# cjcliffe/CubicSDR

Measured on AMD Instinct MI355X. Metric: IQ MS/s sustained @ N demods + FFT size, higher is better.
Workload: dtype f32; 1 GPU; C3: 256 mixed NBFM/AM/USB demods, 61.44 MS/s complex-float IQ, firpfbch M=122, 65536-pt spectrum FFT (internal 131072) over every sample; blocks_per_batch=128, block_len=1024068, n_demods=256, fft_size=65536, audio_samples_per_batch=26215768, streams=1

## Files before the change

cubicsdr_amd/csrc/csdr_bank.hip:

```cpp
#include <algorithm>
#include <cstdlib>
#include <cmath>
#include <map>
#include <memory>

#define CSDR_TU_BANK 1
#include "csdr_objects.hpp"
#include "kernels_fms.hpp"

using namespace csdr;

static int bank_arm_bank(csdr_bank *b, const design::MsresampPlan &p, int *idx) {
    uint32_t key;
    memcpy(&key, &p.rate_arb, 4);
    auto it = b->arm_index.find(key);
    if (it != b->arm_index.end()) { *idx = it->second; return CSDR_OK; }
    const int i = (int)b->arm_index.size();
    b->arms_host.insert(b->arms_host.end(), p.arms.begin(), p.arms.end());
    const size_t need = b->arms_host.size();
    if (need > b->arms.cap) {
        if (int rc = b->ctx->sync_all()) return rc;
        if (int rc = b->arms.reserve(std::max(need, b->arms.cap * 2 + (size_t)kArms * kArmTaps * 8))) return rc;
        CSDR_HIP_TRY(hipMemcpy(b->arms.p, b->arms_host.data(), need * sizeof(float), hipMemcpyHostToDevice));
    } else {
        CSDR_HIP_TRY(hipMemcpy(b->arms.p + (size_t)i * kArms * kArmTaps, p.arms.data(), p.arms.size() * sizeof(float), hipMemcpyHostToDevice));
    }
    b->arm_index[key] = i;
    *idx = i;
    return CSDR_OK;
}

extern "C" int csdr_bank_create(csdr_ctx *ctx, int max_demods, int max_blocks, csdr_bank **out) {
    DeviceScope dev__(ctx);
    if (!ctx || !out || max_demods <= 0 || max_blocks <= 0) return fail(CSDR_EINVAL, "bad argument");
    std::unique_ptr<csdr_bank> b(new csdr_bank());
    b->ctx = ctx; b->max_demods = max_demods; b->max_blocks = max_blocks;
    b->slots.resize(max_demods);
    if (int rc = b->cfgs.reserve(max_demods)) return rc;
    b->off_lists = ((size_t)max_demods * sizeof(SlotDyn) + 15) & ~(size_t)15;
    b->off_plans = (b->off_lists + (6 * (size_t)max_demods + 8 * 32) * sizeof(int) + 15) & ~(size_t)15;
    b->table_bytes = (b->off_plans + (size_t)max_demods * (max_blocks + 1) * sizeof(BlockPlan) + 255) & ~(size_t)255;
// ... 437 lines not shown
    }
    CSDR_HIP_TRY(hipEventRecord(b->stage_ev[ring], fetch_on_post ? c->lanes[LANE_POST] : st));
    b->stage_used[ring] = true;
    if (fetch_on_post) CSDR_HIP_TRY(hipStreamWaitEvent(st, b->stage_ev[ring], 0));
    else if (post->ctx != c || !c->same(LANE_POST, LANE_FE)) {
        if (post->ctx != c) CSDR_HIP_TRY(hipEventRecord(post->ev_ready[pk], post->ctx->lanes[LANE_POST]));
        CSDR_HIP_TRY(hipStreamWaitEvent(st, post->ev_ready[pk], 0));
    }
    const int64_t total = (int64_t)NB * Bc;
    const int fe_slots = std::max(1, c->wg_slots(demod_frontend_s<5, 2048, true>, kFeThreads + 64, fes_lds_bytes<5, 2048>()));
    auto ranges_for = [&](int n_slots) {
        int P = (int)std::max<int64_t>(1, std::min<int64_t>(total / std::max<int64_t>(4096, 4 * (int64_t)warm_max), 4096));
        const int per_slot = fe_slots / std::max(1, n_slots) - 1;
        if (per_slot >= 1) {
            P = std::max(P, (int)std::min<int64_t>(total / std::max<int64_t>(2048, (int64_t)warm_max), 4096));
            P = std::min(P, per_slot);
        }
        else {
            const int rounds = (n_slots * 2 + fe_slots - 1) / fe_slots;
            P = std::max(1, std::min(P, rounds * fe_slots / std::max(1, n_slots) - 1));
        }
        return P;
    };
    size_t fe_lds = 0;
    for (int i = 0; i < grp_n[0]; ++i) fe_lds = std::max(fe_lds, fe_lds_bytes((int)b->slots[grp_h[grp_off[0] + i]].iq.S));
    const int cap_stream = (max_n_iq_ag + kSsbWarm + 64 + 3) & ~3;
    const int cap_cw = max_cw_audio ? ((max_cw_audio + 4 * kHilbM + 64 + 3) & ~3) : 0;
    bool any_dsb = false;
    for (int i = 0; i < n_ag; ++i) any_dsb = any_dsb || b->slots[ag_list_h[i]].prm.modem == CSDR_MODEM_DSB;
    const size_t dsb_lds = any_dsb ? 1024 * sizeof(float) + (size_t)(max_n_iq_ag + 64) * sizeof(float2) : 0;
    const size_t cw_lds = cap_cw ? ((size_t)kCwIqWin + 2 * (size_t)cap_cw) * sizeof(float2) : 0;
    const size_t modem_lds = std::max(std::max((size_t)4 * cap_stream * sizeof(float), cw_lds), dsb_lds) + 64;
    int hist_need = 2 * kArmTaps;
    for (int i = 0; i < n_run; ++i) {
        const SlotHost &s = b->slots[slot_list_h[i]];
        if (is_fe_only(s.prm.modem) || s.prm.modem == CSDR_MODEM_IQ) continue;
        const int aS = (int)s.au.S;
        int64_t lo = 0, need;
        if (s.au.interp) {
            for (int st = aS - 1; st >= 0; --st) lo = (lo >> 1) - (2 * (int)s.au.m[st] - 1);
            need = ((-lo * (int64_t)s.au.step) >> 24) + kArmTaps + 8;
        } else {
            lo = -(int64_t)(kArmTaps - 1);
            for (int e = aS - 1; e >= 0; --e) lo = 2 * lo - (4 * (int)s.au.m[aS - 1 - e] - 2);
            need = -lo + (1 << aS) + 8;
        }
        hist_need = std::max<int>(hist_need, (int)need);
    }
    const int cap_win = (max_n_iq + std::min(hist_need, kDHist) + 64 + 3) & ~3;
    const int cap_out = (std::max(max_n_audio + 32 * max_aS + 64, cap_win / 2 + 64) + 3) & ~3;
    const size_t audio_lds = (size_t)(2 * cap_out + cap_win) * sizeof(float) + 64;
    constexpr size_t kLdsPerWorkgroup = 160 * 1024;
    if (modem_lds > kLdsPerWorkgroup || audio_lds > kLdsPerWorkgroup)
        return reject(fail(CSDR_EUNSUPPORTED, "%d IQ / %d audio samples per block need %zu / %zu bytes of LDS (limit %zu)", max_n_iq, max_n_audio, modem_lds, audio_lds, kLdsPerWorkgroup));
    const int fms_blk = (max_n_iq_fms + 4 * kHilbM + 4 + 3) & ~3, fms_au = (max_n_au_fms + 4 + 3) & ~3;
    const size_t fms_pre_lds = (size_t)fms_blk * sizeof(float), fms_pll_lds = 1024 * sizeof(float) + (size_t)fms_blk * (sizeof(float2) + sizeof(uint32_t)),
                 fms_mix_lds = (size_t)2 * (fms_blk + 4 * kHilbM) * sizeof(float),
                 fms_out_lds = ((size_t)2 * (fms_au + kFmsFirMax) + kFmsFirMax) * sizeof(float) + 64;
    if (n_fms && std::max(std::max(fms_pre_lds, fms_pll_lds), std::max(fms_mix_lds, fms_out_lds)) > kLdsPerWorkgroup)
        return reject(fail(CSDR_EUNSUPPORTED, "FM stereo: %d IQ samples per block need more LDS than a workgroup has", max_n_iq_fms));
    const bool fused1 = NB == 1 && n_fms == 0;
    const size_t want[8] = {fe_lds, modem_lds, audio_lds, n_fms ? fms_pre_lds : 0, n_fms ? fms_pll_lds : 0, n_fms ? fms_mix_lds : 0, n_fms ? fms_out_lds : 0,
                            fused1 ? std::max(modem_lds, audio_lds) : 0};
    const void *fn[8] = {(const void *)demod_frontend, (const void *)demod_modem, (const void *)demod_audio_interp,
                         (const void *)fms_pre, (const void *)fms_pll, (const void *)fms_mix, (const void *)fms_out, (const void *)demod_modem_audio1};
    for (int k = 0; k < 8; ++k)
        if (want[k] > 64 * 1024 && want[k] > b->lds_attr[k]) {
            CSDR_HIP_TRY(hipFuncSetAttribute(fn[k], hipFuncAttributeMaxDynamicSharedMemorySize, (int)want[k]));
            b->lds_attr[k] = want[k];
        }
    const dim3 grid(std::max(1, n_audio_run), NB);
    const int audio_threads = kAudioThreads;
    const float2 *chan_out = post_buf(post, pk);
    const int *grp_d = lists_d + 2 * (size_t)b->max_demods;
    if (grp_n[0] > 0)
        CSDR_LAUNCH(c, LANE_FE, KID_FE_GENERIC, demod_frontend, dim3(ranges_for(grp_n[0]), grp_n[0]), dim3(kFeThreads), fe_lds, b->cfgs.p, dyns_d, grp_d + grp_off[0],
                    chan_out, post->chan_stride, total, b->arms.p, c->sintab.p);
#define CSDR_FE_S(S_, CH_)                                                                                                              \
    if (grp_n[S_] > 0)                                                                                                                  \
        CSDR_LAUNCH(c, LANE_FE, KID_FE_S##S_, (demod_frontend_s<S_, CH_>), dim3(16, grp_rows[S_] * (ranges_for(grp_n[S_]) + 1)), dim3(kFeThreads), (fes_lds_bytes<S_, CH_>()), \
                    b->cfgs.p, dyns_d, grp_d + grp_off[S_], chan_out, post->chan_stride, total, b->arms.p, c->sintab.p, grp_rows[S_])
    CSDR_FE_S(3, 2048); CSDR_FE_S(4, 2048);
    if (grp_n[6] > 0) {
        if (merged56)
            CSDR_LAUNCH(c, LANE_FE, KID_FE_S56, (demod_frontend_s56<2048>), dim3(16, grp_rows[6] * (ranges_for(grp_n[6]) + 1)), dim3(kFeThreads + 64), (fes_lds_bytes<6, 2048>()),
                        b->cfgs.p, dyns_d, grp_d + grp_off[6], chan_out, post->chan_stride, total, b->arms.p, c->sintab.p, grp_rows[6]);
        else
            CSDR_LAUNCH(c, LANE_FE, KID_FE_S6, (demod_frontend_s<6, 2048, true>), dim3(16, grp_rows[6] * (ranges_for(grp_n[6]) + 1)), dim3(kFeThreads + 64), (fes_lds_bytes<6, 2048>()),
                        b->cfgs.p, dyns_d, grp_d + grp_off[6], chan_out, post->chan_stride, total, b->arms.p, c->sintab.p, grp_rows[6]);
    }
    if (grp_n[7] > 0) {
        int64_t jmax = 0;
        for (int i = 0; i < grp_n[7]; ++i) jmax = std::max<int64_t>(jmax, b->slots[grp_h[grp_off[7] + i]].last_J);
        const int nchunks = (int)((jmax + kFiChunk - 1) / kFiChunk);
        CSDR_LAUNCH(c, LANE_FE, KID_FE_INTERP, demod_frontend_interp, dim3(nchunks + 1, grp_n[7]), dim3(kFeThreads), kFiLds, b->cfgs.p, dyns_d, grp_d + grp_off[7],
                    chan_out, post->chan_stride, total, b->arms.p, c->sintab.p);
    }
    if (grp_n[5] > 0)
        CSDR_LAUNCH(c, LANE_FE, KID_FE_S5, (demod_frontend_s<5, 2048, true>), dim3(16, grp_rows[5] * (ranges_for(grp_n[5]) + 1)), dim3(kFeThreads + 64), (fes_lds_bytes<5, 2048>()),
                    b->cfgs.p, dyns_d, grp_d + grp_off[5], chan_out, post->chan_stride, total, b->arms.p, c->sintab.p, grp_rows[5]);
#undef CSDR_FE_S
    CSDR_HIP_TRY(hipGetLastError());
    {
        csdr_post *pw = const_cast<csdr_post *>(post);
        if (pw->ctx != c || !c->same(LANE_POST, LANE_FE)) {
            if (pw->n_consumed[pk] >= csdr_post::kMaxConsumers) return fail(CSDR_ERANGE, "too many demodulator banks read one channelizer batch");
            CSDR_HIP_TRY(hipEventRecord(pw->ev_consumed[pk][pw->n_consumed[pk]++], st));
        }
    }
    if (int rc = c->signal(b->ev_fe_done[bpar], LANE_FE, LANE_AUDIO)) return rc;
    if (int rc = c->wait(b->ev_fe_done[bpar], LANE_FE, LANE_AUDIO)) return rc;
    if (int rc = b->audio.wait(st_a)) return rc;
    if (fused1) {
        if (n_audio_run > 0)
            CSDR_LAUNCH(c, LANE_AUDIO, KID_AUDIO, demod_modem_audio1, dim3(n_audio_run), dim3(audio_threads), std::max(modem_lds, audio_lds), b->cfgs.p, dyns_d, lists_d, plans_d,
                        cap_stream, b->mconsts.p, c->sintab.p, b->arms.p, cap_cw, cap_out, cap_win);
    } else {
    if (n_ag > 0)
        CSDR_LAUNCH(c, LANE_AUDIO, KID_MODEM, demod_modem, dim3(NB, n_ag), dim3(audio_threads) , modem_lds, b->cfgs.p, dyns_d, lists_d + b->max_demods,
                    plans_d, NB, cap_stream, b->mconsts.p, c->sintab.p, b->arms.p, cap_cw);
    if (n_ag > 0 && NB > 1)
        CSDR_LAUNCH(c, LANE_AUDIO, KID_GAIN_SCAN, demod_gain_scan, dim3(n_ag), dim3(64), (size_t)(2 * NB + 1) * sizeof(float), b->cfgs.p, dyns_d, lists_d + b->max_demods, plans_d, NB);
    const int *fms_d = lists_d + b->max_demods + fms_off;
    if (n_fms > 0) {
        CSDR_LAUNCH(c, LANE_AUDIO, KID_FMS, fms_pre, dim3(n_fms, NB), dim3(64), fms_pre_lds, b->cfgs.p, dyns_d, fms_d, plans_d, NB, b->mconsts.p);
        CSDR_LAUNCH(c, LANE_AUDIO, KID_FMS, fms_pll, dim3(n_fms), dim3(kModemThreads), fms_pll_lds, b->cfgs.p, fms_d, plans_d, NB, fms_blk, c->sintab.p);
        CSDR_LAUNCH(c, LANE_AUDIO, KID_FMS, fms_mix, dim3(n_fms, NB), dim3(64), fms_mix_lds, b->cfgs.p, dyns_d, fms_d, plans_d, NB, fms_blk - 4 * kHilbM, b->mconsts.p, c->sintab.p);
    }
    if (n_audio_run > 0)
        CSDR_LAUNCH(c, LANE_AUDIO, KID_AUDIO, demod_audio_interp, grid, dim3(audio_threads), audio_lds, b->cfgs.p, dyns_d, lists_d, plans_d, NB,
                    cap_out, cap_win, b->arms.p, 0);
    if (n_fms > 0) {
        CSDR_LAUNCH(c, LANE_AUDIO, KID_AUDIO, demod_audio_interp, dim3(n_fms, NB), dim3(audio_threads), audio_lds, b->cfgs.p, dyns_d, fms_d, plans_d, NB,
                    cap_out, cap_win, b->arms.p, 1);
        CSDR_LAUNCH(c, LANE_AUDIO, KID_FMS_OUT, fms_out, dim3(n_fms, NB), dim3(64), fms_out_lds, b->cfgs.p, dyns_d, fms_d, plans_d, NB, fms_au);
    }
    }
    if (int rc = bank_digital_launch(b, plans_d, NB)) return rc;
    CSDR_HIP_TRY(hipGetLastError());
    if (int rc = c->signal(b->ev_audio_done[bpar], LANE_AUDIO, LANE_FE)) return rc;
    b->audio_pending[bpar] = true;
    if (fetch_on_post) if (int rc = b->tables_read[bpar].release(st_a)) return rc;
    (void)st_a;
    b->seq++;
    return CSDR_OK;
}

int bank_iq_acquire(csdr_bank *b, hipStream_t reader) {
    if (!b || b->last_nb == 0) return fail(CSDR_ESTATE, "no csdr_bank_execute yet");
    return b->iq[(b->seq - 1) & 1].acquire(b->ctx->lanes[LANE_FE], reader);
}
int bank_iq_release(csdr_bank *b, hipStream_t reader) {
    if (b->seq == 0) return CSDR_OK;
    return b->iq[(b->seq - 1) & 1].release(reader);
}

int bank_audio_acquire(csdr_bank *b, hipStream_t reader) {
    if (!b || b->last_nb == 0) return fail(CSDR_ESTATE, "no csdr_bank_execute yet");
    return b->audio.acquire(b->ctx->lanes[LANE_AUDIO], reader);
}
int bank_audio_release(csdr_bank *b, hipStream_t reader) { return b->audio.release(reader); }
int bank_plan_release(csdr_bank *b, hipStream_t reader) {
    if (b->seq == 0) return CSDR_OK;
    return b->plan[(b->seq - 1) & 1].release(reader);
}

extern "C" int csdr_bank_fetch_results(csdr_bank *b, int slot, csdr_block_result *out, int cap_blocks, int *n_blocks) {
// ... 32 lines not shown
}
extern "C" int csdr_bank_fetch_iq(csdr_bank *b, int slot, float *host_out, int cap_samples, int *n) {
    DeviceScope dev__(b ? b->ctx : nullptr);
    if (!b || !host_out || !n || slot < 0 || slot >= b->max_demods) return fail(CSDR_EINVAL, "bad argument");
    SlotHost &s = b->slots[slot];
    if (s.last_J > cap_samples) return fail(CSDR_ERANGE, "need room for %d samples", s.last_J);
    *n = s.last_J;
    if (s.last_J) {
        const float2 *cur = s.cfg.iq + (size_t)s.last_parity * ((size_t)kIqHist + s.cfg.cap_iq) + kIqHist;
        hipStream_t st = b->ctx->lanes[LANE_FE];
        CSDR_HIP_TRY(hipMemcpyAsync(host_out, cur, (size_t)s.last_J * sizeof(float2), hipMemcpyDeviceToHost, st));
        CSDR_HIP_TRY(hipStreamSynchronize(st));
    }
    return CSDR_OK;
}
extern "C" int csdr_bank_fetch_demod_output(csdr_bank *b, int slot, float *host_out, int cap_samples, int *n) {
    DeviceScope dev__(b ? b->ctx : nullptr);
    if (!b || !host_out || !n || slot < 0 || slot >= b->max_demods) return fail(CSDR_EINVAL, "bad argument");
    SlotHost &s = b->slots[slot];
    *n = 0;
    if (!s.configured || s.last_A == 0 || s.prm.modem == CSDR_MODEM_IQ || s.prm.modem == CSDR_MODEM_CW || s.prm.modem == CSDR_MODEM_FMS) return CSDR_OK;
    hipStream_t st = b->ctx->lanes[LANE_AUDIO];
    int32_t cnt = 0;
    CSDR_HIP_TRY(hipMemcpyAsync(&cnt, s.cfg.scope_n, sizeof cnt, hipMemcpyDeviceToHost, st));
    CSDR_HIP_TRY(hipStreamSynchronize(st));
    cnt = std::min<int32_t>(cnt, cap_samples);
    if (cnt > 0) {
        CSDR_HIP_TRY(hipMemcpyAsync(host_out, s.cfg.scope, (size_t)cnt * sizeof(float), hipMemcpyDeviceToHost, st));
        CSDR_HIP_TRY(hipStreamSynchronize(st));
    }
    *n = cnt;
    return CSDR_OK;
}
extern "C" int csdr_design_fms_pilot(int64_t sample_rate, float *b15, float *a15) {
    if (!b15 || !a15 || sample_rate <= 0) return fail(CSDR_EINVAL, "bad argument");
    const std::vector<design::Sos> sos = design::fms_pilot_sos(sample_rate);
    for (int q = 0; q < 5; ++q) for (int k = 0; k < 3; ++k) { b15[3 * q + k] = sos[q].b[k]; a15[3 * q + k] = sos[q].a[k]; }
    return CSDR_OK;
}
extern "C" int csdr_bank_set_fms_pilot(csdr_bank *b, int slot, const float *b15, const float *a15) {
    DeviceScope dev__(b ? b->ctx : nullptr);
    if (!b || slot < 0 || slot >= b->max_demods) return fail(CSDR_EINVAL, "bad slot");
    SlotHost &s = b->slots[slot];
    if (!s.configured || s.prm.modem != CSDR_MODEM_FMS) return fail(CSDR_ESTATE, "slot %d is not an FM-stereo demodulator", slot);
    if (int rc = b->ctx->sync_all()) return rc;
    if (b15 && a15) { memcpy(s.fms_b, b15, sizeof s.fms_b); memcpy(s.fms_a, a15, sizeof s.fms_a); s.fms_sos_set = true; }
    else {
        s.fms_sos_set = false;
        const std::vector<design::Sos> sos = design::fms_pilot_sos(s.prm.bandwidth);
        for (int q = 0; q < 5; ++q) for (int k = 0; k < 3; ++k) { s.fms_b[3 * q + k] = sos[q].b[k]; s.fms_a[3 * q + k] = sos[q].a[k]; }
    }
    memcpy(s.cfg.fms_b, s.fms_b, sizeof s.fms_b); memcpy(s.cfg.fms_a, s.fms_a, sizeof s.fms_a);
    CSDR_HIP_TRY(hipMemcpy(b->cfgs.p + slot, &s.cfg, sizeof s.cfg, hipMemcpyHostToDevice));
    return CSDR_OK;
}
extern "C" int csdr_bank_fetch_fms_stage(csdr_bank *b, int slot, int which, void *host_out, int cap_samples, int *n) {
    DeviceScope dev__(b ? b->ctx : nullptr);
    if (!b || !host_out || !n || slot < 0 || slot >= b->max_demods || which < 0 || which > 1) return fail(CSDR_EINVAL, "bad argument");
    SlotHost &s = b->slots[slot];
    if (!s.configured || s.prm.modem != CSDR_MODEM_FMS) return fail(CSDR_ESTATE, "slot %d is not an FM-stereo demodulator", slot);
    if (s.last_J > cap_samples) return fail(CSDR_ERANGE, "need room for %d samples", s.last_J);
    *n = s.last_J;
    if (s.last_J) {
        hipStream_t st = b->ctx->lanes[LANE_AUDIO];
        CSDR_HIP_TRY(hipMemcpyAsync(host_out, which == 0 ? (const void *)s.cfg.fms_theta : (const void *)s.cfg.d, (size_t)s.last_J * 4, hipMemcpyDeviceToHost, st));
        CSDR_HIP_TRY(hipStreamSynchronize(st));
// ... 12 lines not shown
```

cubicsdr_amd/csrc/kernels_demod.hpp:

```cpp
#pragma once
#include "common.hpp"
#include "cpx.hpp"

namespace csdr {

constexpr int kMaxHb = 10;
constexpr int kHbMaxM = 10;
constexpr int kArmTaps = 14;
constexpr int kArms = 256;
constexpr int kMixHist = 65536;
constexpr int kIqHist = 1024;
constexpr int kDHist = 1024;
constexpr int kScopeMax = 2048;
constexpr int kFeThreads = 256;
constexpr int kFeChunk = 2048;
constexpr int kFePairs = kFeChunk / 2 / kFeThreads;
constexpr int kFeTail = 24;
constexpr int kFeZTail = 16;

struct ResampCfg {
    int32_t interp;
    int32_t S;
    int32_t m_x[kMaxHb];
    float h_x[kMaxHb][kHbMaxM];
// ... 945 lines not shown
            for (int i = tid; i < nb; i += nthr) s_x[i] = iq[jb + i];
            __syncthreads();
            if (tid == 0) {
                float mx = 0.0f;
                for (int i = 0; i < nb; ++i) {
                    const float2 x = s_x[i];
                    const unsigned idx = (th + (1u << 21)) >> 22;
                    const float sn = s_tab[idx & 1023], cs = s_tab[(idx + 256) & 1023];
                    const float vr = __fadd_rn(__fmul_rn(x.x, cs), __fmul_rn(x.y, sn));
                    const float vi = __fsub_rn(__fmul_rn(x.y, cs), __fmul_rn(x.x, sn));
                    const float e = vr > 0.0f ? vi : -vi;
                    dth += nco_phase_word_dev(alpha * e);
                    th += nco_phase_word_dev(beta * e);
                    th += dth;
                    const float y = vr / 0.5f;
                    d[jb + i] = y;
                    mx = fmaxf(mx, y);
                }
                cfg.blockmax[bb] = mx;
                cfg.bout[bb].level_accum = 0.0; cfg.bout[bb].level_count = 0; cfg.bout[bb].audio_peak = 0.f;
                if (NB == 1) gain_step_single(cfg, dyn, pl, mx);
            }
        }
        if (tid == 0) { cfg.pll[0] = th; cfg.pll[1] = dth; }
        return;
    } else if (cfg.modem == CSDR_MODEM_CW) {
        const ResampCfg &au = cfg.rs_au;
        const int aS = au.S, H = 4 * kHilbM;
        const int64_t A0 = (int64_t)pl[b].q0 << aS, A1 = (int64_t)pl[b + 1].q0 << aS;
        const int n_audio = (int)(A1 - A0);
        float2 *s_iq = reinterpret_cast<float2 *>(smem);
        float2 *w0 = s_iq + kCwIqWin, *w1 = w0 + cap_cw;
        const float *arms = arms_all + (size_t)au.arms_idx * kArms * kArmTaps;
        int64_t lo[kMaxHb + 1], hi[kMaxHb + 1];
        lo[aS] = A0 - H; hi[aS] = A1;
        for (int st = aS - 1; st >= 0; --st) { lo[st] = (lo[st + 1] >> 1) - (2 * au.m_x[st] - 1); hi[st] = (hi[st + 1] + 1) >> 1; }
        const int nv = (int)(hi[0] - lo[0]);
        const int64_t jlo = (((int64_t)dyn.aphase0 + lo[0] * (int64_t)au.step) >> 24) - (kArmTaps - 1);
        const int64_t jhi = nv > 0 ? (((int64_t)dyn.aphase0 + (hi[0] - 1) * (int64_t)au.step) >> 24) + 1 : jlo;
        const int nwin = (int)(jhi - jlo);
        for (int i = tid; i < nwin; i += nthr) {
            const int64_t j = jlo + i;
            s_iq[i] = j >= -(int64_t)kIqHist ? iq[j] : make_float2(0.f, 0.f);
        }
        __syncthreads();
        for (int i = tid; i < nv; i += nthr) {
            const int64_t P = (int64_t)dyn.aphase0 + (lo[0] + i) * (int64_t)au.step;
            const float *h = arms + (int)((P & 0xFFFFFF) >> 16) * kArmTaps;
            const float2 *z = s_iq + ((P >> 24) - (kArmTaps - 1) - jlo);
            float ar = 0.f, ai = 0.f;
#pragma unroll
            for (int t = 0; t < kArmTaps; ++t) { ar = fmaf(h[t], z[t].x, ar); ai = fmaf(h[t], z[t].y, ai); }
            w0[i] = make_float2(ar, ai);
        }
        __syncthreads();
        float2 *src = w0, *dst = w1;
        for (int st = 0; st < aS; ++st) {
            const int m = au.m_x[st];
            const int64_t olo = lo[st + 1], ilo = lo[st];
            const int nout = (int)(hi[st + 1] - olo);
            const int qoff = (int)((olo >> 1) - ilo), par0 = (int)(olo & 1);
            for (int i = tid; i < nout; i += nthr) {
                const int a = i + par0, qi = qoff + (a >> 1);
                float2 v;
                if ((a & 1) == 0) v = src[qi - m];
                else {
                    v = make_float2(0.f, 0.f);
                    for (int j = 0; j < m; ++j) {
                        const float hj = au.h_x[st][j];
                        const float2 p = src[qi - j], q2 = src[qi - (2 * m - 1) + j];
                        v.x = fmaf(hj, p.x + q2.x, v.x); v.y = fmaf(hj, p.y + q2.y, v.y);
                    }
                }
                dst[i] = v;
            }
            __syncthreads();
            float2 *t = src; src = dst; dst = t;
        }
        for (int i = tid; i < n_audio + H; i += nthr) {
            const int64_t a = A0 - H + i;
            float sn, cs;
            nco_sincos(sintab, dyn.ssb_theta0 + (uint32_t)a * dyn.cw_dtheta, sn, cs);
            const float2 v = src[i];
            src[i] = make_float2(v.x * cs - v.y * sn, v.y * cs + v.x * sn);
        }
        __syncthreads();
        for (int i = tid; i < n_audio; i += nthr) {
            const int k = i + H;
            const float yi = src[k - 2 * kHilbM].x;
            float yq = 0.f;
#pragma unroll
            for (int t = 0; t < 2 * kHilbM; ++t) yq = fmaf(mc->hilb60[t], src[k - (2 * t + 1)].y, yq);
            const float v = yi - yq;
            cfg.audio[A0 + i] = v;
// ... 20 lines not shown
            for (int k = 0; k < kSsbFir; ++k) acc = cpx_fma_s(mc->ssb_fir[k], s_ab[i - k], acc);
            s_cd[i] = acc;
        }
        __syncthreads();
        for (int i = kSsbWarm + tid; i < tot; i += nthr) {
            const int j = j0 - pre + i;
            float s, c;
            nco_sincos(sintab, dyn.ssb_theta0 + (uint32_t)(j + 1) * (1u << 30), s, c);
            const float xr = s_cd[i].x, xi = s_cd[i].y;
            s_cd[i] = usb ? cpx_make(xr * c - xi * s, xi * c + xr * s) : cpx_make(xr * c + xi * s, xi * c - xr * s);
        }
        __syncthreads();
        for (int i = tid; i < n; i += nthr) {
            const int k = i + pre;
            const float yi = s_cd[k - 2 * kHilbM].x;
            float yq = 0.f;
#pragma unroll
            for (int t = 0; t < 2 * kHilbM; ++t) yq = fmaf(mc->hilb[t], s_cd[k - (2 * t + 1)].y, yq);
            const float v = usb ? (yi - yq) : (yi + yq);
            d[j0 + i] = v;
            lmax = fmaxf(lmax, v);
        }
    }
    const float bm = wave_max_float(lmax);
    const double bs = wave_sum_double(lsum);
    if (tid == 0) {
        cfg.blockmax[b] = bm;
        cfg.bout[b].level_accum = bs;
        cfg.bout[b].level_count = lcount;
        cfg.bout[b].audio_peak = 0.f;
        if (NB == 1) gain_step_single(cfg, dyn, pl, bm);
    }
}
CSDR_KERNEL_BANK __launch_bounds__(kAudioThreads) void demod_modem(
    const SlotCfg *__restrict__ cfgs, const SlotDyn *__restrict__ dyns, const int *__restrict__ slot_list,
    const BlockPlan *__restrict__ plans, int NB, int cap_stream, const ModemConsts *__restrict__ mc, const float *__restrict__ sintab,
    const float *__restrict__ arms_all, int cap_cw) {
    demod_modem_body(cfgs, dyns, slot_list[blockIdx.y], (int)blockIdx.x, plans, NB, cap_stream, mc, sintab, arms_all, cap_cw);
}

CSDR_KERNEL_BANK __launch_bounds__(64) void demod_gain_scan(const SlotCfg *__restrict__ cfgs, const SlotDyn *__restrict__ dyns, const int *__restrict__ slot_list,
                                                      const BlockPlan *__restrict__ plans, int NB) {
    extern __shared__ __attribute__((aligned(16))) char smem[];
    float *s_max = reinterpret_cast<float *>(smem);
    int *s_j0 = reinterpret_cast<int *>(s_max + NB);
    const int slot = slot_list[blockIdx.x], tid = threadIdx.x;
    const SlotCfg &cfg = cfgs[slot];
    const SlotDyn dyn = dyns[slot];
    const BlockPlan *pl = plans + (size_t)slot * (NB + 1);
    for (int i = tid; i < NB; i += 64) s_max[i] = cfg.blockmax[i];
    for (int i = tid; i <= NB; i += 64) s_j0[i] = pl[i].j0;
    __syncthreads();
    const float *agc_in = cfg.agc + 4 * dyn.hist_parity;
    float ceil_ = agc_in[0], ma = agc_in[1], maa = agc_in[2];
    if (tid == 0)
        for (int bb = 0; bb < NB; ++bb) {
            const float mx = s_max[bb];
            if (s_j0[bb + 1] != s_j0[bb]) {
                ma = ma + (ceil_ - ma) * 0.025f;
                maa = maa + (ma - maa) * 0.025f;
                ceil_ = mx;
            }
            s_max[bb] = maa;
        }
    __syncthreads();
    for (int i = tid; i < NB; i += 64) cfg.blockmaa[i] = s_max[i];
    if (tid != 0) return;
    float *agc_out = cfg.agc + 4 * (dyn.hist_parity ^ 1);
    agc_out[0] = ceil_; agc_out[1] = ma; agc_out[2] = maa;
}

template <int M>
__device__ __forceinline__ void audio_x2_stage(const float *__restrict__ h, const float *__restrict__ src, float *__restrict__ dst, int qoff, int par0, int nout, int tid,
                                               int m_any = 0) {
    constexpr int NT = M ? M : kHbMaxM;
    const int m = M ? M : m_any;
    float hs[NT];
#pragma unroll
    for (int j = 0; j < NT; ++j) hs[j] = h[j];
    for (int p = tid; 2 * p - par0 < nout; p += kAudioThreads) {
        const int qi = qoff + p, i0 = 2 * p - par0;
        const float ve = src[qi - m];
        float vo = 0.f;
#pragma unroll
        for (int j = 0; j < NT; ++j)
            if (M || j < m) vo = fmaf(hs[j], src[qi - j] + src[qi - (2 * m - 1) + j], vo);
        if (i0 >= 0) dst[i0] = ve;
        if (i0 + 1 < nout) dst[i0 + 1] = vo;
    }
}

constexpr int kAudioMaxOut = 16384;

__device__ __forceinline__ void demod_audio_body(
    const SlotCfg *__restrict__ cfgs, const SlotDyn *__restrict__ dyns, const int slot, const int b,
    const BlockPlan *__restrict__ plans, int NB, int cap_out, int cap_win, const float *__restrict__ arms_all, int pass) {
    extern __shared__ __attribute__((aligned(16))) char smem[];
    float *s_w0 = reinterpret_cast<float *>(smem);
    float *s_w1 = s_w0 + cap_out;
    float *s_d = s_w1 + cap_out;

    const int tid = threadIdx.x;
    constexpr int nthr = kAudioThreads;
    const SlotCfg &cfg = cfgs[slot];
    const SlotDyn dyn = dyns[slot];
    const BlockPlan *pl = plans + (size_t)slot * (NB + 1);
    const ResampCfg &au = cfg.rs_au;
    const int aS = au.S;
    const int64_t Q0 = pl[b].q0, Q1 = pl[b + 1].q0;
    const bool interp = au.interp != 0;
    const int64_t A0 = interp ? (Q0 << aS) : Q0, A1 = interp ? (Q1 << aS) : Q1;
    const int n_audio = (int)(A1 - A0);
    const float *arms = arms_all + (size_t)au.arms_idx * kArms * kArmTaps;
    const bool fms = cfg.modem == CSDR_MODEM_FMS, plain = fms && pass == 1;
    const bool autogain = !(cfg.modem == CSDR_MODEM_NBFM || cfg.modem == CSDR_MODEM_FM || fms);
    const float2 *iq = cfg.iq + (size_t)dyn.hist_parity * ((size_t)kIqHist + cfg.cap_iq) + kIqHist;
    if (cfg.modem == CSDR_MODEM_CW) {
        const float maa = cfg.blockmaa[b];
        const float gain_db = 10.0f * log10f(0.5f / maa);
        const float g = powf(10.0f, gain_db / 10.0f);
        const int aS = cfg.rs_au.S;
        const int a0 = pl[b].q0 << aS, n_audio = (pl[b + 1].q0 << aS) - a0;
        float lpk = 0.f;
        double lsum = 0.0;
        for (int i = tid; i < n_audio; i += nthr) {
            const float v = cfg.audio[a0 + i] * g;
            cfg.audio[a0 + i] = v;
            lpk = fmaxf(lpk, fabsf(v));
            lsum += (double)fabsf(v);
        }
        const float pk = wave_max_float(lpk);
        const double sm = wave_sum_double(lsum);
        if (tid == 0) {
            cfg.bout[b].audio_peak = pk; cfg.bout[b].level_accum = sm; cfg.bout[b].level_count = n_audio;
        }
        return;
    }
    if (cfg.modem == CSDR_MODEM_IQ) {
        const int j0 = pl[b].j0, n_iq = pl[b + 1].j0 - j0;
        float lpk = 0.f;
        double lsum = 0.0;
        float2 *ao = reinterpret_cast<float2 *>(cfg.audio) + j0;
        for (int i = tid; i < n_iq; i += nthr) {
            const float2 x = iq[j0 + i];
            ao[i] = make_float2(x.y, x.x);
            lpk = fmaxf(lpk, fmaxf(fabsf(x.x), fabsf(x.y)));
            lsum += sqrt((double)x.x * (double)x.x + (double)x.y * (double)x.y);
        }
        const float pk = wave_max_float(lpk);
        const double sm = wave_sum_double(lsum);
        if (tid == 0) { cfg.bout[b].audio_peak = pk; cfg.bout[b].level_accum = sm; cfg.bout[b].level_count = n_iq; }
        return;
    }
    const float fm_ref = 1.0f / (2.0f * 3.14159265358979323846f * 0.5f);
    const float *dh_in = cfg.dh + (size_t)kDHist * dyn.hist_parity;

    float g_cur = 1.0f, g_prev = 1.0f;
    if (autogain) {
        g_cur = 0.5f / cfg.blockmaa[b];
        if (b > 0) g_prev = 0.5f / cfg.blockmaa[b - 1];
    }

    int64_t lo[kMaxHb + 1], hi[kMaxHb + 1];
    int64_t jlo, jhi;
    int nv = 0;
    if (interp) {
        lo[aS] = A0;
        for (int s = aS - 1; s >= 0; --s) lo[s] = (lo[s + 1] >> 1) - (2 * au.m_x[s] - 1);
        hi[aS] = A1;
        for (int s = aS - 1; s >= 0; --s) hi[s] = (hi[s + 1] + 1) >> 1;
        nv = (int)(hi[0] - lo[0]);
        jlo = (((int64_t)dyn.aphase0 + lo[0] * (int64_t)au.step) >> 24) - (kArmTaps - 1);
        jhi = nv > 0 ? (((int64_t)dyn.aphase0 + (hi[0] - 1) * (int64_t)au.step) >> 24) + 1 : jlo;
    } else {
        lo[aS] = (((int64_t)dyn.aphase0 + Q0 * (int64_t)au.step) >> 24) - (kArmTaps - 1);
        hi[aS] = n_audio > 0 ? (((int64_t)dyn.aphase0 + (Q1 - 1) * (int64_t)au.step) >> 24) + 1 : lo[aS];
        for (int e = aS - 1; e >= 0; --e) { lo[e] = 2 * lo[e + 1] - (4 * au.m_x[e] - 2); hi[e] = 2 * hi[e + 1] - 1; }
        jlo = lo[0] - (int64_t)dyn.abuf0;
        jhi = hi[0] > lo[0] ? hi[0] - (int64_t)dyn.abuf0 : jlo;
    }

    const int nwin = (int)(jhi - jlo);
    const int jb0 = pl[b].j0, jbp = b > 0 ? pl[b - 1].j0 : 0;
    const bool fast_gain = pl[b + 1].j0 > jb0 && (b == 0 || jb0 > jbp);
    auto demod_sample = [&](int64_t j) -> float {
        if (plain) return j < 0 ? (j >= -(int64_t)kDHist ? dh_in[kDHist + j] : 0.f) : cfg.d[j];
        if (!autogain) {
            if (j < -(int64_t)(kIqHist - 1)) return 0.f;
            const float2 c = iq[j], p = iq[j - 1];
            return atan2f(c.y * p.x - c.x * p.y, c.x * p.x + c.y * p.y) * fm_ref;
        }
        if (j < 0) return j >= -(int64_t)kDHist ? dh_in[kDHist + j] : 0.f;
        if (fast_gain && j >= jb0) return cfg.d[j] * g_cur;
        if (fast_gain && j >= jbp) return cfg.d[j] * g_prev;
        int bb = b;
        while (bb > 0 && j < pl[bb].j0) --bb;
        return cfg.d[j] * (0.5f / cfg.blockmaa[bb]);
    };
    if (!plain && !autogain) {
        const int64_t jmin = -(int64_t)(kIqHist - 1);
        for (int i0 = tid; i0 < nwin; i0 += 4 * nthr) {
            float2 c4[4], p4[4];
#pragma unroll
            for (int u = 0; u < 4; ++u) {
                const int64_t j = jlo + min(i0 + u * nthr, nwin - 1);
                const int64_t jc = j < jmin ? jmin : j;
                c4[u] = iq[jc]; p4[u] = iq[jc - 1];
            }
#pragma unroll
            for (int u = 0; u < 4; ++u) {
                const int i = i0 + u * nthr;
                const float2 c = c4[u], pq = p4[u];
                const float v = atan2f(c.y * pq.x - c.x * pq.y, c.x * pq.x + c.y * pq.y) * fm_ref;
                if (i < nwin) s_d[i] = (jlo + i) < jmin ? 0.f : v;
            }
        }
    } else
    for (int i = tid; i < nwin; i += nthr) s_d[i] = demod_sample(jlo + i);
    if (b == NB - 1 && !fms) {
        const int n_own = pl[b + 1].j0 - jb0;
        const int ns = max(0, min(n_own, kScopeMax));
        const int staged = max(0, min(ns, (int)(jhi - (int64_t)jb0)));
        __syncthreads();
        for (int i = tid; i < ns; i += nthr) cfg.scope[i] = (i < staged && (int64_t)jb0 >= jlo) ? s_d[(int)((int64_t)jb0 - jlo) + i] : demod_sample((int64_t)jb0 + i);
        if (tid == 0) *cfg.scope_n = ns;
    }
    float2 hv[2][kArmTaps / 2];
    int zoff[2] = {0, 0};
    float *src = s_w0, *dst = s_w1;
    if (interp) {
#pragma unroll
    for (int r = 0; r < 2; ++r) {
        const int i = tid + r * nthr;
        if (i < nv) {
            const int64_t P = (int64_t)dyn.aphase0 + (lo[0] + i) * (int64_t)au.step;
            zoff[r] = (int)((P >> 24) - (kArmTaps - 1) - jlo);
            const float2 *h2 = reinterpret_cast<const float2 *>(arms + (int)((P & 0xFFFFFF) >> 16) * kArmTaps);
#pragma unroll
            for (int t = 0; t < kArmTaps / 2; ++t) hv[r][t] = h2[t];
        }
    }
    __syncthreads();
#pragma unroll
    for (int r = 0; r < 2; ++r) {
        const int i = tid + r * nthr;
        if (i < nv) {
            const float *z = s_d + zoff[r];
            float acc = 0.f;
#pragma unroll
            for (int t = 0; t < kArmTaps / 2; ++t) { acc = fmaf(hv[r][t].x, z[2 * t], acc); acc = fmaf(hv[r][t].y, z[2 * t + 1], acc); }
            s_w0[i] = acc;
        }
    }
    for (int i0 = tid + 2 * nthr; i0 < nv; i0 += 2 * nthr) {
        float2 ha[2][kArmTaps / 2];
        int zo[2];
#pragma unroll
        for (int r = 0; r < 2; ++r) {
            const int i = min(i0 + r * nthr, nv - 1);
            const int64_t P = (int64_t)dyn.aphase0 + (lo[0] + i) * (int64_t)au.step;
            zo[r] = (int)((P >> 24) - (kArmTaps - 1) - jlo);
            const float2 *h2 = reinterpret_cast<const float2 *>(arms + (int)((P & 0xFFFFFF) >> 16) * kArmTaps);
#pragma unroll
            for (int t = 0; t < kArmTaps / 2; ++t) ha[r][t] = h2[t];
        }
#pragma unroll
        for (int r = 0; r < 2; ++r) {
            const int i = i0 + r * nthr;
            const float *z = s_d + zo[r];
            float acc = 0.f;
#pragma unroll
            for (int t = 0; t < kArmTaps / 2; ++t) { acc = fmaf(ha[r][t].x, z[2 * t], acc); acc = fmaf(ha[r][t].y, z[2 * t + 1], acc); }
            if (i < nv) s_w0[i] = acc;
        }
    }
    __syncthreads();
    for (int s = 0; s < aS; ++s) {
        const int m = au.m_x[s];
        const int64_t olo = lo[s + 1], ohi = hi[s + 1], ilo = lo[s];
        const int nout = (int)(ohi - olo);
        const int qoff = (int)((olo >> 1) - ilo), par0 = (int)(olo & 1);
        switch (m) {
            case 3: audio_x2_stage<3>(au.h_x[s], src, dst, qoff, par0, nout, tid); break;
            case 5: audio_x2_stage<5>(au.h_x[s], src, dst, qoff, par0, nout, tid); break;
            case 10: audio_x2_stage<10>(au.h_x[s], src, dst, qoff, par0, nout, tid); break;
            default: audio_x2_stage<0>(au.h_x[s], src, dst, qoff, par0, nout, tid, m); break;
        }
        __syncthreads();
        float *t = src; src = dst; dst = t;
    }
    } else {
        __syncthreads();
        const float *in = s_d;
        float *ping = s_w0, *pong = s_w1;
        const float zeta = 1.0f / (float)(1 << aS);
        for (int e = 0; e < aS; ++e) {
            const int m = au.m_x[e];
            const int64_t ilo = lo[e], olo = lo[e + 1];
            const int nout = (int)(hi[e + 1] - olo);
            const float sc = (e == aS - 1) ? zeta : 1.0f;
            float hs[kHbMaxM];
#pragma unroll
            for (int j = 0; j < kHbMaxM; ++j) hs[j] = au.h_x[e][j];
            const int xoff = (int)(2 * olo - ilo);
            for (int i = tid; i < nout; i += nthr) {
                const float *x = in + (xoff + 2 * i);
                float v = x[-2 * m + 1];
#pragma unroll
                for (int j = 0; j < kHbMaxM; ++j)
                    if (j < m) v = fmaf(hs[j], x[-2 * j] + x[-4 * m + 2 + 2 * j], v);
                ping[i] = v * sc;
            }
            __syncthreads();
            in = ping;
            float *t = ping; ping = pong; pong = t;
        }
        for (int i = tid; i < n_audio; i += nthr) {
            const int64_t P = (int64_t)dyn.aphase0 + (Q0 + i) * (int64_t)au.step;
            const int64_t kq = P >> 24;
            const float *h = arms + (int)((P & 0xFFFFFF) >> 16) * kArmTaps;
            const float *z = in + (kq - (kArmTaps - 1) - lo[aS]);
            float acc = 0.f;
#pragma unroll
            for (int t = 0; t < kArmTaps; ++t) acc = fmaf(h[t], z[t], acc);
            ping[i] = acc;
        }
        __syncthreads();
        src = ping;
    }
    float lpk = 0.f;
    double lsum = 0.0;
    const int aoff = (int)A0;
    float *aout = fms ? (pass ? cfg.fms_s : cfg.fms_m) : cfg.audio;
    for (int i = tid; i < n_audio; i += nthr) {
        const float v = src[i];
        aout[aoff + i] = v;
        lpk = fmaxf(lpk, fabsf(v));
        if (autogain) lsum += (double)fabsf(v);
    }
    const int n_iq = pl[b + 1].j0 - jb0;
    if (!autogain && !plain)
        for (int i = tid; i < n_iq; i += nthr) {
            const float2 x = iq[jb0 + i];
            lsum += sqrt((double)x.x * (double)x.x + (double)x.y * (double)x.y);
        }
    const float pk = wave_max_float(lpk);
    const double sm = wave_sum_double(lsum);
    if (tid == 0 && !plain) {
        cfg.bout[b].audio_peak = pk;
        cfg.bout[b].level_accum = sm;
        cfg.bout[b].level_count = autogain ? n_audio : n_iq;
    }
    if (b == NB - 1 && (autogain || plain)) {
        const int J = pl[NB].j0;
        for (int td = tid; td < kDHist; td += nthr) {
            const int j = J - kDHist + td;
            float dv;
            if (j < 0) dv = dh_in[kDHist + j];
            else if (plain) dv = cfg.d[j];
            else if (fast_gain && j >= jb0) dv = cfg.d[j] * g_cur;
            else if (fast_gain && j >= jbp) dv = cfg.d[j] * g_prev;
            else {
                int bb = b;
                while (bb > 0 && j < pl[bb].j0) --bb;
                dv = cfg.d[j] * (0.5f / cfg.blockmaa[bb]);
            }
            (cfg.dh + (size_t)kDHist * (dyn.hist_parity ^ 1))[td] = dv;
        }
    }
}
CSDR_KERNEL_BANK __launch_bounds__(kAudioThreads) void demod_audio_interp(
    const SlotCfg *__restrict__ cfgs, const SlotDyn *__restrict__ dyns, const int *__restrict__ slot_list,
    const BlockPlan *__restrict__ plans, int NB, int cap_out, int cap_win, const float *__restrict__ arms_all, int pass) {
    demod_audio_body(cfgs, dyns, slot_list[blockIdx.x], (int)blockIdx.y, plans, NB, cap_out, cap_win, arms_all, pass);
}

CSDR_KERNEL_BANK __launch_bounds__(kAudioThreads) void demod_modem_audio1(
    const SlotCfg *__restrict__ cfgs, const SlotDyn *__restrict__ dyns, const int *__restrict__ slot_list, const BlockPlan *__restrict__ plans,
    int cap_stream, const ModemConsts *__restrict__ mc, const float *__restrict__ sintab, const float *__restrict__ arms_all, int cap_cw,
    int cap_out, int cap_win) {
    const int slot = slot_list[blockIdx.x];
    const int modem = cfgs[slot].modem;
    if (modem == CSDR_MODEM_AM || modem == CSDR_MODEM_USB || modem == CSDR_MODEM_LSB || modem == CSDR_MODEM_DSB || modem == CSDR_MODEM_CW) {
        demod_modem_body(cfgs, dyns, slot, 0, plans, 1, cap_stream, mc, sintab, arms_all, cap_cw);
#if defined(__AMDGCN__)
        __builtin_amdgcn_fence(__ATOMIC_SEQ_CST, "workgroup");
        __builtin_amdgcn_s_dcache_inv();
#endif
        __syncthreads();
    }
    demod_audio_body(cfgs, dyns, slot, 0, plans, 1, cap_out, cap_win, arms_all, 0);
}

}
```

Baseline: 74700 MS/s.

## Shrink audio LDS arena and drop per-stage range arrays to raise occupancy

Interpolating audio slots now use a single arena whose size comes from a tighter host-side rule, and the halfband stages ping-pong between its two ends instead of using three separate buffers. The goal is less dynamic LDS per workgroup. The per-level lo/hi int64 arrays are replaced by a lambda that recomputes each range on demand, which cuts register and scratch use. Launch bounds now request 5 waves per EU on the modem and audio kernels. In exchange, range math is recomputed at every stage, the arena overlap has to be exactly right or outputs get corrupted, and a debug gain-trace API is added.

```diff
diff --git a/cubicsdr_amd/csrc/audio_lds_rule.hpp b/cubicsdr_amd/csrc/audio_lds_rule.hpp
--- /dev/null
+++ b/cubicsdr_amd/csrc/audio_lds_rule.hpp
@@ -0,0 +1,18 @@
+#pragma once
+#include <algorithm>
+#include <cstdint>
+
+namespace csdr {
+
+inline int64_t audio_arena_floats(int64_t n_audio_max, int aS, const int *m, uint32_t step, int taps) {
+    int64_t n_out = n_audio_max, need = 0;
+    for (int s = aS - 1; s >= 0; --s) {
+        const int64_t n_in = (n_out >> 1) + 2 * (int64_t)m[s];
+        need = std::max(need, n_in + n_out);
+        n_out = n_in;
+    }
+    const int64_t nwin = ((n_out * (int64_t)step) >> 24) + taps + 2;
+    return std::max(need, nwin + n_out);
+}
+
+}
diff --git a/cubicsdr_amd/csrc/csdr_bank.hip b/cubicsdr_amd/csrc/csdr_bank.hip
--- a/cubicsdr_amd/csrc/csdr_bank.hip
+++ b/cubicsdr_amd/csrc/csdr_bank.hip
@@ -7,6 +7,7 @@
 #define CSDR_TU_BANK 1
 #include "csdr_objects.hpp"
 #include "kernels_fms.hpp"
+#include "audio_lds_rule.hpp"
 
 using namespace csdr;
 
@@ -510,10 +511,21 @@
     const size_t cw_lds = cap_cw ? ((size_t)kCwIqWin + 2 * (size_t)cap_cw) * sizeof(float2) : 0;
     const size_t modem_lds = std::max(std::max((size_t)4 * cap_stream * sizeof(float), cw_lds), dsb_lds) + 64;
     int hist_need = 2 * kArmTaps;
+    int64_t arena_need = 0;
+    bool any_decim = false;
     for (int i = 0; i < n_run; ++i) {
         const SlotHost &s = b->slots[slot_list_h[i]];
         if (is_fe_only(s.prm.modem) || s.prm.modem == CSDR_MODEM_IQ) continue;
         const int aS = (int)s.au.S;
+        if (s.prm.modem != CSDR_MODEM_CW) {
+            if (s.au.interp) {
+                const bool fms = s.prm.modem == CSDR_MODEM_FMS;
+                int blk = 0, mm[kMaxHb];
+                for (const csdr_block_result &r : s.results) blk = std::max(blk, fms ? r.n_audio / 2 : r.n_audio);
+                for (int st = 0; st < aS; ++st) mm[st] = (int)s.au.m[st];
+                arena_need = std::max(arena_need, audio_arena_floats(blk, aS, mm, s.au.step, kArmTaps));
+            } else any_decim = true;
+        }
         int64_t lo = 0, need;
         if (s.au.interp) {
             for (int st = aS - 1; st >= 0; --st) lo = (lo >> 1) - (2 * (int)s.au.m[st] - 1);
@@ -527,7 +539,8 @@
     }
     const int cap_win = (max_n_iq + std::min(hist_need, kDHist) + 64 + 3) & ~3;
     const int cap_out = (std::max(max_n_audio + 32 * max_aS + 64, cap_win / 2 + 64) + 3) & ~3;
-    const size_t audio_lds = (size_t)(2 * cap_out + cap_win) * sizeof(float) + 64;
+    const int cap_arena = (int)((arena_need + 3) & ~(int64_t)3);
+    const size_t audio_lds = (size_t)std::max(any_decim ? 2 * cap_out + cap_win : 0, cap_arena) * sizeof(float) + 64;
     constexpr size_t kLdsPerWorkgroup = 160 * 1024;
     if (modem_lds > kLdsPerWorkgroup || audio_lds > kLdsPerWorkgroup)
         return reject(fail(CSDR_EUNSUPPORTED, "%d IQ / %d audio samples per block need %zu / %zu bytes of LDS (limit %zu)", max_n_iq, max_n_audio, modem_lds, audio_lds, kLdsPerWorkgroup));
@@ -592,7 +605,7 @@
     if (fused1) {
         if (n_audio_run > 0)
             CSDR_LAUNCH(c, LANE_AUDIO, KID_AUDIO, demod_modem_audio1, dim3(n_audio_run), dim3(audio_threads), std::max(modem_lds, audio_lds), b->cfgs.p, dyns_d, lists_d, plans_d,
-                        cap_stream, b->mconsts.p, c->sintab.p, b->arms.p, cap_cw, cap_out, cap_win);
+                        cap_stream, b->mconsts.p, c->sintab.p, b->arms.p, cap_cw, cap_out, cap_win, cap_arena);
     } else {
     if (n_ag > 0)
         CSDR_LAUNCH(c, LANE_AUDIO, KID_MODEM, demod_modem, dim3(NB, n_ag), dim3(audio_threads) , modem_lds, b->cfgs.p, dyns_d, lists_d + b->max_demods,
@@ -607,10 +620,10 @@
     }
     if (n_audio_run > 0)
         CSDR_LAUNCH(c, LANE_AUDIO, KID_AUDIO, demod_audio_interp, grid, dim3(audio_threads), audio_lds, b->cfgs.p, dyns_d, lists_d, plans_d, NB,
-                    cap_out, cap_win, b->arms.p, 0);
+                    cap_out, cap_win, cap_arena, b->arms.p,0);
     if (n_fms > 0) {
         CSDR_LAUNCH(c, LANE_AUDIO, KID_AUDIO, demod_audio_interp, dim3(n_fms, NB), dim3(audio_threads), audio_lds, b->cfgs.p, dyns_d, fms_d, plans_d, NB,
-                    cap_out, cap_win, b->arms.p, 1);
+                    cap_out, cap_win, cap_arena, b->arms.p,1);
         CSDR_LAUNCH(c, LANE_AUDIO, KID_FMS_OUT, fms_out, dim3(n_fms, NB), dim3(64), fms_out_lds, b->cfgs.p, dyns_d, fms_d, plans_d, NB, fms_au);
     }
     }
@@ -709,6 +722,20 @@
     *n = cnt;
     return CSDR_OK;
 }
+extern "C" int csdr_bank_debug_gain_trace(csdr_bank *b, int slot, float *blockmax, float *blockmaa, int cap_blocks, float *agc_in3, float *agc_out3) {
+    DeviceScope dev__(b ? b->ctx : nullptr);
+    if (!b || !blockmax || !blockmaa || !agc_in3 || !agc_out3 || slot < 0 || slot >= b->max_demods) return fail(CSDR_EINVAL, "bad argument");
+    SlotHost &s = b->slots[slot];
+    if (!s.configured || b->last_nb <= 0 || b->last_nb > cap_blocks) return fail(CSDR_ESTATE, "slot %d: nothing to report, or more blocks than the caller has room for", slot);
+    hipStream_t st = b->ctx->lanes[LANE_AUDIO];
+    float agc[8];
+    CSDR_HIP_TRY(hipMemcpyAsync(blockmax, s.cfg.blockmax, (size_t)b->last_nb * sizeof(float), hipMemcpyDeviceToHost, st));
+    CSDR_HIP_TRY(hipMemcpyAsync(blockmaa, s.cfg.blockmaa, (size_t)b->last_nb * sizeof(float), hipMemcpyDeviceToHost, st));
+    CSDR_HIP_TRY(hipMemcpyAsync(agc, s.cfg.agc, sizeof agc, hipMemcpyDeviceToHost, st));
+    CSDR_HIP_TRY(hipStreamSynchronize(st));
+    for (int k = 0; k < 3; ++k) { agc_in3[k] = agc[4 * s.last_parity + k]; agc_out3[k] = agc[4 * (s.last_parity ^ 1) + k]; }
+    return CSDR_OK;
+}
 extern "C" int csdr_design_fms_pilot(int64_t sample_rate, float *b15, float *a15) {
     if (!b15 || !a15 || sample_rate <= 0) return fail(CSDR_EINVAL, "bad argument");
     const std::vector<design::Sos> sos = design::fms_pilot_sos(sample_rate);
diff --git a/cubicsdr_amd/csrc/kernels_demod.hpp b/cubicsdr_amd/csrc/kernels_demod.hpp
--- a/cubicsdr_amd/csrc/kernels_demod.hpp
+++ b/cubicsdr_amd/csrc/kernels_demod.hpp
@@ -1001,12 +1001,15 @@
         float2 *s_iq = reinterpret_cast<float2 *>(smem);
         float2 *w0 = s_iq + kCwIqWin, *w1 = w0 + cap_cw;
         const float *arms = arms_all + (size_t)au.arms_idx * kArms * kArmTaps;
-        int64_t lo[kMaxHb + 1], hi[kMaxHb + 1];
-        lo[aS] = A0 - H; hi[aS] = A1;
-        for (int st = aS - 1; st >= 0; --st) { lo[st] = (lo[st + 1] >> 1) - (2 * au.m_x[st] - 1); hi[st] = (hi[st + 1] + 1) >> 1; }
-        const int nv = (int)(hi[0] - lo[0]);
-        const int64_t jlo = (((int64_t)dyn.aphase0 + lo[0] * (int64_t)au.step) >> 24) - (kArmTaps - 1);
-        const int64_t jhi = nv > 0 ? (((int64_t)dyn.aphase0 + (hi[0] - 1) * (int64_t)au.step) >> 24) + 1 : jlo;
+        auto range_at = [&](int level, int64_t &l, int64_t &h) {
+            l = A0 - H; h = A1;
+            for (int t = aS - 1; t >= level; --t) { l = (l >> 1) - (2 * au.m_x[t] - 1); h = (h + 1) >> 1; }
+        };
+        int64_t lo0, hi0;
+        range_at(0, lo0, hi0);
+        const int nv = (int)(hi0 - lo0);
+        const int64_t jlo = (((int64_t)dyn.aphase0 + lo0 * (int64_t)au.step) >> 24) - (kArmTaps - 1);
+        const int64_t jhi = nv > 0 ? (((int64_t)dyn.aphase0 + (hi0 - 1) * (int64_t)au.step) >> 24) + 1 : jlo;
         const int nwin = (int)(jhi - jlo);
         for (int i = tid; i < nwin; i += nthr) {
             const int64_t j = jlo + i;
@@ -1014,7 +1017,7 @@
         }
         __syncthreads();
         for (int i = tid; i < nv; i += nthr) {
-            const int64_t P = (int64_t)dyn.aphase0 + (lo[0] + i) * (int64_t)au.step;
+            const int64_t P = (int64_t)dyn.aphase0 + (lo0 + i) * (int64_t)au.step;
             const float *h = arms + (int)((P & 0xFFFFFF) >> 16) * kArmTaps;
             const float2 *z = s_iq + ((P >> 24) - (kArmTaps - 1) - jlo);
             float ar = 0.f, ai = 0.f;
@@ -1026,9 +1029,10 @@
         float2 *src = w0, *dst = w1;
         for (int st = 0; st < aS; ++st) {
             const int m = au.m_x[st];
-            const int64_t olo = lo[st + 1], ilo = lo[st];
-            const int nout = (int)(hi[st + 1] - olo);
-            const int qoff = (int)((olo >> 1) - ilo), par0 = (int)(olo & 1);
+            int64_t olo, ohi;
+            range_at(st + 1, olo, ohi);
+            const int nout = (int)(ohi - olo);
+            const int qoff = 2 * m - 1, par0 = (int)(olo & 1);
             for (int i = tid; i < nout; i += nthr) {
                 const int a = i + par0, qi = qoff + (a >> 1);
                 float2 v;
@@ -1115,7 +1119,7 @@
         if (NB == 1) gain_step_single(cfg, dyn, pl, bm);
     }
 }
-CSDR_KERNEL_BANK __launch_bounds__(kAudioThreads) void demod_modem(
+CSDR_KERNEL_BANK __launch_bounds__(kAudioThreads, 5) void demod_modem(
     const SlotCfg *__restrict__ cfgs, const SlotDyn *__restrict__ dyns, const int *__restrict__ slot_list,
     const BlockPlan *__restrict__ plans, int NB, int cap_stream, const ModemConsts *__restrict__ mc, const float *__restrict__ sintab,
     const float *__restrict__ arms_all, int cap_cw) {
@@ -1177,11 +1181,11 @@
 
 __device__ __forceinline__ void demod_audio_body(
     const SlotCfg *__restrict__ cfgs, const SlotDyn *__restrict__ dyns, const int slot, const int b,
-    const BlockPlan *__restrict__ plans, int NB, int cap_out, int cap_win, const float *__restrict__ arms_all, int pass) {
+    const BlockPlan *__restrict__ plans, int NB, int cap_out, int cap_win, int cap_arena, const float *__restrict__ arms_all, int pass) {
     extern __shared__ __attribute__((aligned(16))) char smem[];
     float *s_w0 = reinterpret_cast<float *>(smem);
     float *s_w1 = s_w0 + cap_out;
-    float *s_d = s_w1 + cap_out;
+    float *s_d = cfgs[slot].rs_au.interp ? s_w0 : s_w1 + cap_out;
 
     const int tid = threadIdx.x;
     constexpr int nthr = kAudioThreads;
@@ -1244,23 +1248,30 @@
         if (b > 0) g_prev = 0.5f / cfg.blockmaa[b - 1];
     }
 
-    int64_t lo[kMaxHb + 1], hi[kMaxHb + 1];
+    int64_t lo_top, hi_top;
+    if (interp) { lo_top = A0; hi_top = A1; }
+    else {
+        lo_top = (((int64_t)dyn.aphase0 + Q0 * (int64_t)au.step) >> 24) - (kArmTaps - 1);
+        hi_top = n_audio > 0 ? (((int64_t)dyn.aphase0 + (Q1 - 1) * (int64_t)au.step) >> 24) + 1 : lo_top;
+    }
+    auto range_at = [&](int level, int64_t &l, int64_t &h) {
+        l = lo_top; h = hi_top;
+        for (int t = aS - 1; t >= level; --t) {
+            if (interp) { l = (l >> 1) - (2 * au.m_x[t] - 1); h = (h + 1) >> 1; }
+            else { l = 2 * l - (4 * au.m_x[t] - 2); h = 2 * h - 1; }
+        }
+    };
+    int64_t lo0, hi0;
+    range_at(0, lo0, hi0);
     int64_t jlo, jhi;
     int nv = 0;
     if (interp) {
-        lo[aS] = A0;
-        for (int s = aS - 1; s >= 0; --s) lo[s] = (lo[s + 1] >> 1) - (2 * au.m_x[s] - 1);
-        hi[aS] = A1;
-        for (int s = aS - 1; s >= 0; --s) hi[s] = (hi[s + 1] + 1) >> 1;
-        nv = (int)(hi[0] - lo[0]);
-        jlo = (((int64_t)dyn.aphase0 + lo[0] * (int64_t)au.step) >> 24) - (kArmTaps - 1);
-        jhi = nv > 0 ? (((int64_t)dyn.aphase0 + (hi[0] - 1) * (int64_t)au.step) >> 24) + 1 : jlo;
+        nv = (int)(hi0 - lo0);
+        jlo = (((int64_t)dyn.aphase0 + lo0 * (int64_t)au.step) >> 24) - (kArmTaps - 1);
+        jhi = nv > 0 ? (((int64_t)dyn.aphase0 + (hi0 - 1) * (int64_t)au.step) >> 24) + 1 : jlo;
     } else {
-        lo[aS] = (((int64_t)dyn.aphase0 + Q0 * (int64_t)au.step) >> 24) - (kArmTaps - 1);
-        hi[aS] = n_audio > 0 ? (((int64_t)dyn.aphase0 + (Q1 - 1) * (int64_t)au.step) >> 24) + 1 : lo[aS];
-        for (int e = aS - 1; e >= 0; --e) { lo[e] = 2 * lo[e + 1] - (4 * au.m_x[e] - 2); hi[e] = 2 * hi[e + 1] - 1; }
-        jlo = lo[0] - (int64_t)dyn.abuf0;
-        jhi = hi[0] > lo[0] ? hi[0] - (int64_t)dyn.abuf0 : jlo;
+        jlo = lo0 - (int64_t)dyn.abuf0;
+        jhi = hi0 > lo0 ? hi0 - (int64_t)dyn.abuf0 : jlo;
     }
 
     const int nwin = (int)(jhi - jlo);
@@ -1310,13 +1321,14 @@
     }
     float2 hv[2][kArmTaps / 2];
     int zoff[2] = {0, 0};
-    float *src = s_w0, *dst = s_w1;
+    float *src = s_w0;
     if (interp) {
+    float *const s_v = s_w0 + (cap_arena - nv);
 #pragma unroll
     for (int r = 0; r < 2; ++r) {
         const int i = tid + r * nthr;
         if (i < nv) {
-            const int64_t P = (int64_t)dyn.aphase0 + (lo[0] + i) * (int64_t)au.step;
+            const int64_t P = (int64_t)dyn.aphase0 + (lo0 + i) * (int64_t)au.step;
             zoff[r] = (int)((P >> 24) - (kArmTaps - 1) - jlo);
             const float2 *h2 = reinterpret_cast<const float2 *>(arms + (int)((P & 0xFFFFFF) >> 16) * kArmTaps);
 #pragma unroll
@@ -1332,7 +1344,7 @@
             float acc = 0.f;
 #pragma unroll
             for (int t = 0; t < kArmTaps / 2; ++t) { acc = fmaf(hv[r][t].x, z[2 * t], acc); acc = fmaf(hv[r][t].y, z[2 * t + 1], acc); }
-            s_w0[i] = acc;
+            s_v[i] = acc;
         }
     }
     for (int i0 = tid + 2 * nthr; i0 < nv; i0 += 2 * nthr) {
@@ -1341,7 +1353,7 @@
 #pragma unroll
         for (int r = 0; r < 2; ++r) {
             const int i = min(i0 + r * nthr, nv - 1);
-            const int64_t P = (int64_t)dyn.aphase0 + (lo[0] + i) * (int64_t)au.step;
+            const int64_t P = (int64_t)dyn.aphase0 + (lo0 + i) * (int64_t)au.step;
             zo[r] = (int)((P >> 24) - (kArmTaps - 1) - jlo);
             const float2 *h2 = reinterpret_cast<const float2 *>(arms + (int)((P & 0xFFFFFF) >> 16) * kArmTaps);
 #pragma unroll
@@ -1354,15 +1366,18 @@
             float acc = 0.f;
 #pragma unroll
             for (int t = 0; t < kArmTaps / 2; ++t) { acc = fmaf(ha[r][t].x, z[2 * t], acc); acc = fmaf(ha[r][t].y, z[2 * t + 1], acc); }
-            if (i < nv) s_w0[i] = acc;
+            if (i < nv) s_v[i] = acc;
         }
     }
     __syncthreads();
+    src = s_v;
     for (int s = 0; s < aS; ++s) {
         const int m = au.m_x[s];
-        const int64_t olo = lo[s + 1], ohi = hi[s + 1], ilo = lo[s];
+        int64_t olo, ohi;
+        range_at(s + 1, olo, ohi);
         const int nout = (int)(ohi - olo);
-        const int qoff = (int)((olo >> 1) - ilo), par0 = (int)(olo & 1);
+        const int qoff = 2 * m - 1, par0 = (int)(olo & 1);
+        float *const dst = (s & 1) ? s_w0 + (cap_arena - nout) : s_w0;
         switch (m) {
             case 3: audio_x2_stage<3>(au.h_x[s], src, dst, qoff, par0, nout, tid); break;
             case 5: audio_x2_stage<5>(au.h_x[s], src, dst, qoff, par0, nout, tid); break;
@@ -1370,7 +1385,7 @@
             default: audio_x2_stage<0>(au.h_x[s], src, dst, qoff, par0, nout, tid, m); break;
         }
         __syncthreads();
-        float *t = src; src = dst; dst = t;
+        src = dst;
     }
     } else {
         __syncthreads();
@@ -1379,13 +1394,14 @@
         const float zeta = 1.0f / (float)(1 << aS);
         for (int e = 0; e < aS; ++e) {
             const int m = au.m_x[e];
-            const int64_t ilo = lo[e], olo = lo[e + 1];
-            const int nout = (int)(hi[e + 1] - olo);
+            int64_t olo, ohi;
+            range_at(e + 1, olo, ohi);
+            const int nout = (int)(ohi - olo);
             const float sc = (e == aS - 1) ? zeta : 1.0f;
             float hs[kHbMaxM];
 #pragma unroll
             for (int j = 0; j < kHbMaxM; ++j) hs[j] = au.h_x[e][j];
-            const int xoff = (int)(2 * olo - ilo);
+            const int xoff = 4 * m - 2;
             for (int i = tid; i < nout; i += nthr) {
                 const float *x = in + (xoff + 2 * i);
                 float v = x[-2 * m + 1];
@@ -1402,7 +1418,7 @@
             const int64_t P = (int64_t)dyn.aphase0 + (Q0 + i) * (int64_t)au.step;
             const int64_t kq = P >> 24;
             const float *h = arms + (int)((P & 0xFFFFFF) >> 16) * kArmTaps;
-            const float *z = in + (kq - (kArmTaps - 1) - lo[aS]);
+            const float *z = in + (kq - (kArmTaps - 1) - lo_top);
             float acc = 0.f;
 #pragma unroll
             for (int t = 0; t < kArmTaps; ++t) acc = fmaf(h[t], z[t], acc);
@@ -1452,16 +1468,16 @@
         }
     }
 }
-CSDR_KERNEL_BANK __launch_bounds__(kAudioThreads) void demod_audio_interp(
+CSDR_KERNEL_BANK __launch_bounds__(kAudioThreads, 5) void demod_audio_interp(
     const SlotCfg *__restrict__ cfgs, const SlotDyn *__restrict__ dyns, const int *__restrict__ slot_list,
-    const BlockPlan *__restrict__ plans, int NB, int cap_out, int cap_win, const float *__restrict__ arms_all, int pass) {
-    demod_audio_body(cfgs, dyns, slot_list[blockIdx.x], (int)blockIdx.y, plans, NB, cap_out, cap_win, arms_all, pass);
-}
-
-CSDR_KERNEL_BANK __launch_bounds__(kAudioThreads) void demod_modem_audio1(
+    const BlockPlan *__restrict__ plans, int NB, int cap_out, int cap_win, int cap_arena, const float *__restrict__ arms_all, int pass) {
+    demod_audio_body(cfgs, dyns, slot_list[blockIdx.x], (int)blockIdx.y, plans, NB, cap_out, cap_win, cap_arena, arms_all, pass);
+}
+
+CSDR_KERNEL_BANK __launch_bounds__(kAudioThreads, 5) void demod_modem_audio1(
     const SlotCfg *__restrict__ cfgs, const SlotDyn *__restrict__ dyns, const int *__restrict__ slot_list, const BlockPlan *__restrict__ plans,
     int cap_stream, const ModemConsts *__restrict__ mc, const float *__restrict__ sintab, const float *__restrict__ arms_all, int cap_cw,
-    int cap_out, int cap_win) {
+    int cap_out, int cap_win, int cap_arena) {
     const int slot = slot_list[blockIdx.x];
     const int modem = cfgs[slot].modem;
     if (modem == CSDR_MODEM_AM || modem == CSDR_MODEM_USB || modem == CSDR_MODEM_LSB || modem == CSDR_MODEM_DSB || modem == CSDR_MODEM_CW) {
@@ -1472,7 +1488,7 @@
 #endif
         __syncthreads();
     }
-    demod_audio_body(cfgs, dyns, slot, 0, plans, 1, cap_out, cap_win, arms_all, 0);
-}
-
-}
+    demod_audio_body(cfgs, dyns, slot, 0, plans, 1, cap_out, cap_win, cap_arena, arms_all, 0);
+}
+
+}
```

Result: no change. 75380 MS/s (median of 6 runs) (+0.9%).
